# r9y9/wavenet_vocoder

Measured on NVIDIA B200. Metric: audio samples/sec (22.05 kHz MoL, 24-layer), higher is better.
Workload: dtype f32

## Files before the change

### wavenet_vocoder_b200/csrc/wn_host.cu

```cuda
#include <cuda_runtime.h>
#include <stdint.h>
#include <stdio.h>
#include <stdlib.h>
#include <string.h>
#include <math.h>

#include <algorithm>
#include <string>
#include <vector>

#include "../../include/wn.h"
#include "wn_plan.h"
#include "wn_kernel.cuh"
#include "wn7_plan.h"
#include "wn7_kernel.cuh"
#include "wn_aux.cuh"

static thread_local std::string g_err;
static int32_t fail(int32_t code, const std::string& msg) {
    g_err = msg;
    return code;
}
#define CUDA_TRY(expr)                                                                          \
    do {                                                                                        \
// ... 60 lines not shown
    pl.O = c.out_channels;
    pl.kw = c.kernel_size;
    pl.C = c.cin_channels;
    pl.gin = c.gin_channels;
    pl.input_kind = c.input_kind;
    pl.head_kind = c.head_kind;
    pl.Kmix = (c.head_kind == WN_HEAD_SOFTMAX) ? 0 : (c.out_channels == 2 ? 1 : c.out_channels / 3);
    pl.skip_scale = (float)sqrt(1.0 / (double)c.layers);
    pl.BT = batch <= 1 ? 1 : (batch <= 2 ? 2 : (batch <= 4 ? 4 : 8));
    const int BT = pl.BT;

    int P = c.num_ctas > 0 ? c.num_ctas : env_int("WN_NUM_CTAS", 0);
    if (P <= 0) {
        const int cap = std::min(num_sms, pl.G2);
        const int per = wn_ceil_div(pl.G2, cap);
        P = wn_ceil_div(pl.G2, per);
    }
    if (P > num_sms) return fail(WN_ERR_INVALID, "num_ctas exceeds the SM count (blocks must be co-resident)");
    if (P > pl.G2) return fail(WN_ERR_INVALID, "num_ctas exceeds gate_channels/2");
    pl.P = P;
    pl.NYm = wn_ceil_div(pl.G2, P);
    pl.NXm = wn_ceil_div(pl.R, P);
    pl.NSm = wn_ceil_div(pl.S, P);
    pl.NAm = wn_ceil_div(pl.S, P);
    pl.NBm = wn_ceil_div(pl.O, P);
    pl.RA = 2 * pl.NYm;
    pl.NQ_A = wn_ceil_div(pl.RA, 4);
    pl.RA4 = 4 * pl.NQ_A;
    pl.NQ_D = wn_ceil_div((pl.kw - 1) * pl.RA, 4);
    pl.NQ_BO = wn_ceil_div(pl.NXm, 4);
    pl.NQ_BS = wn_ceil_div(pl.NSm, 4);
    pl.NQ_HA = wn_ceil_div(pl.NAm, 4);
    pl.NQ_HB = wn_ceil_div(pl.NBm, 4);
    int o = 0;
    pl.fb_Zx = o; o += pl.NQ_A * pl.R * 4;
    pl.fb_zb = o; o += pl.RA4;
    pl.fb_floats = align_up(o, 4);
    o = 0;
    pl.lb_Zy = o; o += pl.NQ_A * pl.G2 * 4;
    pl.lb_Zx = o; o += pl.NQ_A * pl.R * 4;
    pl.lb_Xo = o; o += pl.NQ_BO * pl.G2 * 4;
    pl.lb_Td = o; o += pl.NQ_D * pl.R * 4;
    pl.lb_Sk = o; o += pl.NQ_BS * pl.G2 * 4;
    pl.lb_zb = o; o += pl.RA4;
    pl.lb_xb = o; o += 4 * pl.NQ_BO;
    pl.lb_sb = o; o += 4 * pl.NQ_BS;
    pl.lb_floats = align_up(o, 4);
    o = 0;
    pl.tb_Td = o;  o += pl.NQ_D * pl.R * 4;
    pl.tb_Sk = o;  o += pl.NQ_BS * pl.G2 * 4;
    pl.tb_sb = o;  o += 4 * pl.NQ_BS;
    pl.tb_Ha = o;  o += pl.NQ_HA * pl.S * 4;
    pl.tb_Hab = o; o += 4 * pl.NQ_HA;
    pl.tb_Hb = o;  o += pl.NQ_HB * pl.S * 4;
    pl.tb_Hbb = o; o += 4 * pl.NQ_HB;
    pl.tb_floats = align_up(o, 4);
    pl.slot_floats = align_up(std::max(pl.fb_floats, std::max(pl.L > 1 ? pl.lb_floats : 0, pl.tb_floats)), 32);
    pl.cta_w_floats = (long long)pl.fb_floats + (long long)(pl.L - 1) * pl.lb_floats + pl.tb_floats;
    pl.nblobs = pl.L + 1;
    pl.cta_cw_floats = (long long)pl.L * pl.NQ_A * pl.C * 4;

    pl.NE = pl.L + 3;
    int nc = c.exchange_copies > 0 ? c.exchange_copies : env_int("WN_NCOPY", 0);
    const int max_items = std::max(std::max(pl.NYm, pl.NXm), std::max(pl.NSm, std::max(pl.NAm, pl.NBm))) * BT;
    if (max_items > 64) return fail(WN_ERR_INVALID, "too many rows per block for this batch tile (use more blocks)");
    if (nc <= 0) nc = 1;
// ... 165 lines not shown
    const int R = pl.R, G2 = pl.G2, kw = pl.kw, S = pl.S, L = pl.L;
    auto grow = [&](int rr) { return (rr & 1) ? G2 + y0 + (rr >> 1) : y0 + (rr >> 1); };
    auto pack_taps = [&](float* grp, int layer) {
        const float* cw = w.layers[layer].conv_w;
        for (int rr = 0; rr < 2 * ny; ++rr)
            for (int tap = 0; tap < kw - 1; ++tap)
                for (int k = 0; k < R; ++k)
                    put_q(grp, R, tap * pl.RA + rr, k, cw[(size_t)grow(rr) * kw * R + (size_t)tap * R + k]);
    };
    auto pack_skip = [&](float* grp, float* bias, int layer) {
        const wn_layer_weights& lw = w.layers[layer];
        for (int r = 0; r < ns; ++r) {
            for (int k = 0; k < G2; ++k) put_q(grp, G2, r, k, lw.skip_w[(size_t)(s0 + r) * G2 + k]);
            bias[r] = lw.skip_b ? lw.skip_b[s0 + r] : 0.f;
        }
    };
    {
        float* blob = out;
        for (int rr = 0; rr < 2 * ny; ++rr) {
            for (int k = 0; k < R; ++k) put_q(blob + pl.fb_Zx, R, rr, k, f.V[0][(size_t)grow(rr) * R + k]);
            blob[pl.fb_zb + rr] = f.zb[0][grow(rr)];
        }
    }
    for (int s = 1; s < L; ++s) {
        float* blob = out + wn_blob_off(pl, s);
        const wn_layer_weights& pw = w.layers[s - 1];
        for (int rr = 0; rr < 2 * ny; ++rr) {
            const int g = grow(rr);
            for (int k = 0; k < G2; ++k) put_q(blob + pl.lb_Zy, G2, rr, k, f.M[s - 1][(size_t)g * G2 + k]);
            for (int k = 0; k < R; ++k) put_q(blob + pl.lb_Zx, R, rr, k, f.V[s][(size_t)g * R + k]);
            blob[pl.lb_zb + rr] = f.zb[s][g];
        }
        for (int r = 0; r < nx; ++r) {
            for (int k = 0; k < G2; ++k) put_q(blob + pl.lb_Xo, G2, r, k, pw.out_w[(size_t)(x0 + r) * G2 + k]);
            blob[pl.lb_xb + r] = pw.out_b ? pw.out_b[x0 + r] : 0.f;
        }
        pack_taps(blob + pl.lb_Td, s - 1);
        pack_skip(blob + pl.lb_Sk, blob + pl.lb_sb, s - 1);
    }
    float* tb = out + wn_blob_off(pl, L);
    pack_taps(tb + pl.tb_Td, L - 1);
    pack_skip(tb + pl.tb_Sk, tb + pl.tb_sb, L - 1);
    for (int r = 0; r < na; ++r) {
        const float* row = w.last_a_w + (size_t)(a0 + r) * S;
        for (int k = 0; k < S; ++k) put_q(tb + pl.tb_Ha, S, r, k, row[k]);
        tb[pl.tb_Hab + r] = w.last_a_b ? w.last_a_b[a0 + r] : 0.f;
    }
    for (int r = 0; r < nb; ++r) {
        const float* row = w.last_b_w + (size_t)(b0 + r) * S;
        for (int k = 0; k < S; ++k) put_q(tb + pl.tb_Hb, S, r, k, row[k]);
        tb[pl.tb_Hbb + r] = w.last_b_b ? w.last_b_b[b0 + r] : 0.f;
    }
}

static void pack_cw_cta(const WnPlan& pl, const wn_weights& w, int p, float* out) {
    if (pl.C <= 0) return;
    memset(out, 0, (size_t)pl.cta_cw_floats * sizeof(float));
    int y0, ny;
    wn_part(pl.G2, pl.P, p, y0, ny);
    for (int l = 0; l < pl.L; ++l) {
        const float* cwm = w.layers[l].cond_w;
        float* grp = out + (size_t)l * pl.NQ_A * pl.C * 4;
        for (int j = 0; j < ny; ++j)
            for (int ab = 0; ab < 2; ++ab) {
                const int rr = 2 * j + ab, grow = ab ? pl.G2 + y0 + j : y0 + j;
                for (int ch = 0; ch < pl.C; ++ch) put_q(grp, pl.C, rr, ch, cwm[(size_t)grow * pl.C + ch]);
            }
    }
// ... 130 lines not shown
    pp.T = T;
    pp.T_test = Tt;
    pp.initial_index = a->initial_index < 0 ? 127 : a->initial_index;
    pp.flags = a->flags;
    pp.noise_kind = a->noise_kind;
    pp.seed = a->seed;
    pp.timeout_cycles = (long long)env_int("WN_TIMEOUT_MS", 2000) * 1500000LL;
    pp.warp_reverse = env_int("WN_WARP_REVERSE", 0);
    pp.gate_cycles = env_int("WN_GATE_CYCLES", 0);
    pp.fast_gate = env_int("WN_FAST_GATE", 0);
    pp.prof = nullptr;
    if (env_int("WN_PROF", 0)) {
        const size_t pb = (size_t)pl.P * 16 * sizeof(long long);
        rc = ensure(&h->d_prof, &h->prof_bytes, pb);
        if (rc) return rc;
        CUDA_TRY(cudaMemsetAsync(h->d_prof, 0, pb, st));
        pp.prof = h->d_prof;
    }

    void* kargs[2] = {(void*)&pl, (void*)&pp};
    auto efor = [](int K) { return K <= 128 ? 1 : (K <= 256 ? 2 : (K <= 512 ? 4 : 8)); };
    const int er = efor(pl.R), eg = efor(pl.G2);
    const int var = (er == 1 && eg == 1) ? 0 : ((er <= 2 && eg <= 2) ? 1 : ((er <= 4 && eg <= 2) ? 2 : 3));
    {
        static const int evar[4][2] = {{1, 1}, {2, 2}, {4, 2}, {8, 8}};
        const int chunk = 1 << pl.xc_shift;
        pl.lean = (BT == 1 && (var == 1 || var == 2) && pl.ncopy == 1 && pl.kw == 3 && pl.RA == 4 && pl.NQ_A == 1 && pl.NQ_BO == 1 && pl.NQ_BS == 1 &&
                   pl.NQ_D == 2 && pl.L >= 2 && evar[var][0] * 128 == pl.R && evar[var][1] * 128 == pl.G2 &&
                   (evar[var][0] % 2) == 0 && (evar[var][1] % 2) == 0 && (pl.ex_yx % chunk) == 0 &&
                   ((pl.G2 + pl.R) % chunk) == 0 && (pl.G2 % chunk) == 0 && (pl.xstride % 2) == 0 &&
                   pl.S == pl.G2 && pl.NQ_HA == 1 && pl.NQ_HB == 1 && pl.O <= 128 && (pl.ex_sk % chunk) == 0 &&
                   (pl.ex_h1 % chunk) == 0 &&
                   env_int("WN_LEAN", 0) != 0) ? 1 : 0;
    }
    const void* fn = nullptr;
#define WN_PICK(BT_)                                                                          \
    fn = var == 0 ? (const void*)wn::wn_persistent_kernel<BT_, 1, 1>                          \
       : var == 1 ? (const void*)wn::wn_persistent_kernel<BT_, 2, 2>                          \
       : var == 2 ? (const void*)wn::wn_persistent_kernel<BT_, 4, 2>                          \
                  : (const void*)wn::wn_persistent_kernel<BT_, 8, 8>
    switch (BT) {
        case 1: WN_PICK(1); break;
        case 2: WN_PICK(2); break;
        case 4: WN_PICK(4); break;
        default: WN_PICK(8); break;
    }
#undef WN_PICK
    if (pl.lean)
        fn = var == 1 ? (const void*)wn::wn_persistent_kernel<1, 2, 2, true>
                      : (const void*)wn::wn_persistent_kernel<1, 4, 2, true>;
    const int ai = pl.lean ? 16 + var : bt_index(BT) * 4 + var;
    if (!h->attr_set[ai]) {
        CUDA_TRY(cudaFuncSetAttribute(fn, cudaFuncAttributeMaxDynamicSharedMemorySize, (int)h->smem_cap));
        h->attr_set[ai] = true;
    }
    cudaLaunchConfig_t lc;
    memset(&lc, 0, sizeof(lc));
    lc.gridDim = dim3(pl.P);
    lc.blockDim = dim3(WN_NTHREADS);
    lc.dynamicSmemBytes = (size_t)pl.smem_bytes;
    lc.stream = st;
    cudaLaunchAttribute la[2];
    int na = 0;
    la[na].id = cudaLaunchAttributeCooperative;
    la[na].val.cooperative = 1;
    ++na;
    if (h->l2_mode == 1 && h->l2_persist_bytes > 0 && h->wpack_bytes > 0) {
        const size_t win = std::min(h->wpack_bytes, h->l2_window_max);
        la[na].id = cudaLaunchAttributeAccessPolicyWindow;
        la[na].val.accessPolicyWindow.base_ptr = (void*)h->d_wpack;
        la[na].val.accessPolicyWindow.num_bytes = win;
        la[na].val.accessPolicyWindow.hitRatio = (float)std::min(1.0, (double)h->l2_persist_bytes / (double)win);
        la[na].val.accessPolicyWindow.hitProp = cudaAccessPropertyPersisting;
        la[na].val.accessPolicyWindow.missProp = cudaAccessPropertyStreaming;
        ++na;
    } else if (h->l2_mode == 2 && h->l2_persist_bytes > 0) {
        la[na].id = cudaLaunchAttributeAccessPolicyWindow;
        la[na].val.accessPolicyWindow.base_ptr = (void*)h->d_xbuf;
        la[na].val.accessPolicyWindow.num_bytes = std::min(xb, h->l2_window_max);
        la[na].val.accessPolicyWindow.hitRatio = 1.0f;
        la[na].val.accessPolicyWindow.hitProp = cudaAccessPropertyPersisting;
        la[na].val.accessPolicyWindow.missProp = cudaAccessPropertyNormal;
        ++na;
    }
// ... 740 lines not shown
```

### wavenet_vocoder_b200/csrc/wn_kernel.cuh

```cuda
#pragma once
#include <cuda_runtime.h>
#include <stdint.h>
#include <math.h>
#include "wn_plan.h"

struct WnPtrs {
    const float* wpack;
    const float* cwpack;
    const float* gbias;
    const float* first_w;
    const float* first_b;
    uint2* xbuf;
    float* ring_g;
    const int* ringtab;
    int* err;
    const float* c;
    const float* initial;
    const float* initial_dense;
    const int* initial_rows;
    const float* test_scalar;
    const int* test_index;
    const float* test_dense;
    const float* u1;
    const float* u2;
// ... 37 lines not shown
    asm volatile(
        "{\n\t.reg .pred p;\n\t"
        "mbarrier.try_wait.parity.shared::cta.b64 p, [%1], %2;\n\t"
        "selp.u32 %0, 1, 0, p;\n\t}"
        : "=r"(ok)
        : "r"(smem_u32(bar)), "r"(parity)
        : "memory");
    return ok != 0;
}
__device__ __forceinline__ void bulk_g2s(void* dst, const void* src, uint32_t bytes, uint64_t* bar) {
    asm volatile(
        "cp.async.bulk.shared::cluster.global.mbarrier::complete_tx::bytes [%0], [%1], %2, [%3];" ::"r"(
            smem_u32(dst)),
        "l"(src), "r"(bytes), "r"(smem_u32(bar))
        : "memory");
}
__device__ __forceinline__ uint2 ld_pair(const uint2* p) {
    uint2 v;
    asm volatile("ld.relaxed.gpu.global.v2.u32 {%0,%1}, [%2];" : "=r"(v.x), "=r"(v.y) : "l"(p) : "memory");
    return v;
}
__device__ __forceinline__ uint4 ld_pair2(const uint2* p) {
    uint4 v;
    asm volatile("ld.relaxed.gpu.global.v4.u32 {%0,%1,%2,%3}, [%4];"
                 : "=r"(v.x), "=r"(v.y), "=r"(v.z), "=r"(v.w)
                 : "l"(p)
                 : "memory");
    return v;
}
__device__ __forceinline__ void st_pair(uint2* p, float v, uint32_t tag) {
    asm volatile("st.relaxed.gpu.global.v2.u32 [%0], {%1,%2};" ::"l"(p), "r"(__float_as_uint(v)), "r"(tag)
                 : "memory");
}
__device__ __forceinline__ void fence_cta() { asm volatile("fence.acq_rel.cta;" ::: "memory"); }
__device__ __forceinline__ int ld_flag(const int* p) {
    int v;
    asm volatile("ld.relaxed.gpu.global.s32 %0, [%1];" : "=r"(v) : "l"(p) : "memory");
    return v;
}
__device__ __forceinline__ bool bar_or(bool pred) {
    uint32_t r;
    asm volatile(
        "{\n\t.reg .pred p, q;\n\t"
        "setp.ne.u32 p, %1, 0;\n\t"
        "bar.red.or.pred q, 1, %2, p;\n\t"
        "selp.u32 %0, 1, 0, q;\n\t}"
        : "=r"(r)
        : "r"((uint32_t)pred), "n"(WN_NT)
        : "memory");
    return r != 0;
}

template <int ID, int N>
__device__ __forceinline__ bool bar_or_n(bool pred) {
    uint32_t r;
    asm volatile(
        "{\n\t.reg .pred p, q;\n\t"
        "setp.ne.u32 p, %1, 0;\n\t"
        "bar.red.or.pred q, %2, %3, p;\n\t"
        "selp.u32 %0, 1, 0, q;\n\t}"
        : "=r"(r)
        : "r"((uint32_t)pred), "n"(ID), "n"(N)
        : "memory");
    return r != 0;
}

// ... 112 lines not shown
    }
    return false;
}
__device__ __noinline__ bool wn_wait_bar_slow(uint64_t* bar, uint32_t parity, volatile int* s_abort, int* err,
                                              long long timeout, uint32_t what, int p) {
    uint32_t spins = 0;
    long long t0 = 0;
    while (!mbar_try_wait(bar, parity)) {
        if (((++spins) & 255u) == 0 && wn_check_abort(s_abort, err, timeout, what, p, t0)) return false;
    }
    return true;
}
__device__ __noinline__ bool wn_wait_count_slow(volatile int* cnt, int need, unsigned sleep_ns, volatile int* s_abort,
                                                int* err, long long timeout, uint32_t what, int p) {
    uint32_t spins = 0;
    long long t0 = 0;
    while (*cnt < need) {
        if (sleep_ns) __nanosleep(sleep_ns);
        if (((++spins) & 63u) == 0 && wn_check_abort(s_abort, err, timeout, what, p, t0)) return false;
    }
    return true;
}

#define WN_NTC 128
#define WN_GW 4
#define WN_DISPATCH_E(EV, ...)                                \
    switch (EV) {                                             \
        case 1: { constexpr int E = 1; __VA_ARGS__ } break;   \
        case 2: { constexpr int E = 2; __VA_ARGS__ } break;   \
        case 4: { constexpr int E = 4; __VA_ARGS__ } break;   \
        default: { constexpr int E = 8; __VA_ARGS__ } break;  \
    }

template <int BT, int ER, int EG, bool LEAN = false>
struct Engine {
    static_assert(!LEAN || (BT == 1 && ER % 2 == 0 && EG % 2 == 0), "lean path: one utterance, paired elements");
    static constexpr int NV = 4 * BT;
    static constexpr int NA = (BT >= 8) ? 1 : 2;
    const WnPlan& pl;
    const WnPtrs& pp;
    unsigned char* sm;
    int tid, warp, lane, p;
    int gt, gw;
    uint64_t *bar_full, *bar_empty, *bar_cfull, *bar_cempty;
    volatile int* s_abort;
    volatile int* s_stash_cnt;
    volatile int* s_ddone_cnt;
    int* ringtab;
    float *xs, *ys, *red1, *red2, *sb, *pre, *cond, *skipacc, *hs, *noise, *first, *slots;
    volatile float* ring;
    float* s_in;
    int* s_idx;
    float* s_dense;
    bool dead;

    __device__ Engine(const WnPlan& pl_, const WnPtrs& pp_, unsigned char* sm_)
        : pl(pl_), pp(pp_), sm(sm_) {
        lane = threadIdx.x & 31;
        warp = pp.warp_reverse ? (WN_NTHREADS / 32 - 1) - (int)(threadIdx.x >> 5) : (int)(threadIdx.x >> 5);
        tid = warp * 32 + lane;
        p = blockIdx.x;
        gt = tid & (WN_NTC - 1);
        gw = warp & (WN_GW - 1);
        const int nslots = pl.nres + pl.nring;
        bar_full = reinterpret_cast<uint64_t*>(sm + pl.sm_bar);
        bar_empty = bar_full + nslots;
        bar_cfull = bar_empty + (pl.nring > 0 ? pl.nring : 1);
        bar_cempty = bar_cfull + 2;
        s_abort = reinterpret_cast<volatile int*>(sm + pl.sm_misc);
// ... 96 lines not shown
#pragma unroll
                    for (int b = 0; b < BT; ++b) x[j][b] = 0.f;
                }
            }
        }
        return bad;
    }
    template <int E>
    __device__ __forceinline__ void poll_vec(const uint2* __restrict__ src, int e0, int K, uint32_t tag,
                                             float (&x)[E][BT]) {
        uint32_t spins = 0;
        long long t0 = 0;
        while (load_vec<E>(src, e0, K, tag, x) != 0) {
            if (((++spins) & 63u) == 0 && check_abort(tag, t0)) {
                dead = true;
                return;
            }
        }
    }
    template <int EA, int EB>
    __device__ __forceinline__ void poll_vec2(const uint2* __restrict__ src, int ea, int KA, float (&a)[EA][BT],
                                              int eb, int KB, float (&b)[EB][BT], uint32_t tag) {
        uint32_t spins = 0;
        long long t0 = 0;
        while (true) {
            const uint32_t bad = load_vec<EA>(src, ea, KA, tag, a) | load_vec<EB>(src, eb, KB, tag, b);
            if (bad == 0) return;
            if (((++spins) & 63u) == 0 && check_abort(tag, t0)) {
                dead = true;
                return;
            }
        }
    }
    template <int E>
    __device__ __forceinline__ void stash(float* dst, int K, const float (&x)[E][BT]) {
#pragma unroll
        for (int j = 0; j < E; ++j) {
            const int k = elem<E>(j);
            if (k < K) {
#pragma unroll
                for (int b = 0; b < BT; ++b) dst[k * BT + b] = x[j][b];
            }
        }
    }
    template <int E>
    __device__ __forceinline__ void unstash(const float* src, int K, float (&x)[E][BT]) {
#pragma unroll
        for (int j = 0; j < E; ++j) {
            const int k = elem<E>(j);
#pragma unroll
            for (int b = 0; b < BT; ++b) x[j][b] = (k < K) ? src[k * BT + b] : 0.f;
        }
    }

    template <int E>
    __device__ __forceinline__ void quad_fma(const float* __restrict__ wq , int K,
                                             const float (&x)[E][BT], float (&acc)[NV]) {
#pragma unroll
        for (int j = 0; j < E; ++j) {
            const int k = elem<E>(j);
            if (k < K) {
                const float4 w4 = *reinterpret_cast<const float4*>(wq + (size_t)k * 4);
#pragma unroll
                for (int b = 0; b < BT; ++b) {
                    acc[0 * BT + b] = fmaf(w4.x, x[j][b], acc[0 * BT + b]);
                    acc[1 * BT + b] = fmaf(w4.y, x[j][b], acc[1 * BT + b]);
// ... 382 lines not shown
            if (lane == 0) mbar_arrive(&bar_cempty[t & 1]);
        }
    }

    __device__ void crit_loop() {
        const int L = pl.L, R = pl.R, G2 = pl.G2, S = pl.S, O = pl.O, T = pp.T, P = pl.P, ncopy = pl.ncopy;
        int y0, ny, x0r, nx, s0, ns, a0, na, b0, nb;
        wn_part(G2, P, p, y0, ny);
        wn_part(R, P, p, x0r, nx);
        wn_part(S, P, p, s0, ns);
        wn_part(S, P, p, a0, na);
        wn_part(O, P, p, b0, nb);
        const int ES = efor(S), EO = efor(O);
        const uint2* xin = pp.xbuf + (size_t)(p % ncopy) * pl.copy_stride_pairs;
        const uint32_t NEID = (uint32_t)L + 3u;
        const int YX = G2 + R;
        const float RSQRT2 = 0.70710678118654752440f;
        const int NQ_A = pl.NQ_A, NQ_BO = pl.NQ_BO, nqc = NQ_A + NQ_BO;
        const int fl = gt & 63;
        const bool grpA = gt < 64;
        auto role = [&](int nitems, int& item, int& copy) {
            item = -1; copy = 0;
            if (nitems > 0 && fl < nitems * ncopy) { item = fl % nitems; copy = fl / nitems; }
        };
        int it_y, cp_y, it_x, cp_x, it_s, cp_s, it_a, cp_a, it_b, cp_b;
        role(ny * BT, it_y, cp_y);
        role(nx * BT, it_x, cp_x);
        role(ns * BT, it_s, cp_s);
        role(na * BT, it_a, cp_a);
        role(nb * BT, it_b, cp_b);
        if (!grpA) it_y = it_s = it_a = it_b = -1;
        if (grpA) it_x = -1;
        const int pa_idx = it_y >= 0 ? (2 * (it_y / BT)) * BT + (it_y % BT) : 0;
        float xr[ER][BT], yr[EG][BT];
        const bool prof = (pp.prof != nullptr) && tid == 0;
        long long pc[8] = {0, 0, 0, 0, 0, 0, 0, 0}, tc = 0;
#define WN_TICK(i) if (prof) { const long long now_ = clock64(); pc[i] += now_ - tc; tc = now_; }
        int nstash = 0;
        int ndone = 0;
        long long t_pub = clock64();
        if (bar_groups(false)) return;

        constexpr bool LEAN_T = LEAN;
        constexpr bool lean = LEAN;
        constexpr int LY = LEAN_T ? EG / 2 : 1, LX = LEAN_T ? ER / 2 : 1;
        long long lk_y[LY], lk_x[LX], l_inc = 0;
        const uint2* l_in0 = xin;
        uint2 *l_puby = pp.xbuf, *l_pubx = pp.xbuf;
        const float* l_pre = pre;
        const uint2 *l_sk0 = xin, *l_h10 = xin;
        uint2 *l_pubs = pp.xbuf, *l_puba = pp.xbuf, *l_pubb = pp.xbuf;
        int l_zy = 0, l_zx = 0, l_xo = 0, l_redw = 0, l_reda = 0, l_redx = 0, l_xb = 0, l_xs = 0;
#pragma unroll
        for (int j = 0; j < LY; ++j) lk_y[j] = 0;
#pragma unroll
        for (int j = 0; j < LX; ++j) lk_x[j] = 0;
        if (lean) {
#pragma unroll
            for (int j = 0; j < LY; ++j) lk_y[j] = wn_pair_index((long long)(2 * gt + 2 * WN_NTC * j));
#pragma unroll
            for (int j = 0; j < LX; ++j) lk_x[j] = wn_pair_index((long long)(G2 + 2 * gt + 2 * WN_NTC * j));
            l_inc = wn_pair_index((long long)YX);
            l_in0 = xin + wn_pair_index((long long)pl.ex_yx);
            l_puby = pp.xbuf + wn_pair_index((long long)pl.ex_yx) + wn_pair_index((long long)(y0 + max(it_y, 0)));
            l_pubx = pp.xbuf + wn_pair_index((long long)pl.ex_yx) + wn_pair_index((long long)(G2 + x0r + max(it_x, 0)));
            l_pre = pre + 2 * max(it_y, 0);
            l_zy = pl.lb_Zy + 8 * gt;
            l_zx = pl.lb_Zx + 8 * gt;
            l_xo = pl.lb_Xo + 8 * gt;
            l_redw = (lane >> 2) * WN_GW + gw;
            l_reda = 2 * max(it_y, 0) * WN_GW;
            l_redx = (4 + max(it_x, 0)) * WN_GW;
            l_xb = pl.lb_xb + max(it_x, 0);
            l_xs = x0r + max(it_x, 0);
            l_sk0 = xin + wn_pair_index((long long)pl.ex_sk);
            l_h10 = xin + wn_pair_index((long long)pl.ex_h1);
            l_pubs = pp.xbuf + wn_pair_index((long long)(pl.ex_sk + s0 + max(it_s, 0)));
            l_puba = pp.xbuf + wn_pair_index((long long)(pl.ex_h1 + a0 + max(it_a, 0)));
            l_pubb = pp.xbuf + wn_pair_index((long long)(pl.ex_h2 + b0 + max(it_b, 0)));
        }
        auto lean_poll_y = [&](const uint2* base, uint32_t tag) {
            uint4 ry[LY];
            uint32_t need = (1u << LY) - 1u, spins = 0;
            while (true) {
#pragma unroll
                for (int j = 0; j < LY; ++j)
                    if (need & (1u << j)) ry[j] = ld_pair2(base + lk_y[j]);
#pragma unroll
                for (int j = 0; j < LY; ++j)
                    if (((ry[j].y ^ tag) | (ry[j].w ^ tag)) == 0u) need &= ~(1u << j);
                if (need == 0u) break;
                if (((++spins) & 63u) == 0 && wn_poll_check(s_abort, pp.err, spins, pp.timeout_cycles, tag, p)) {
                    dead = true;
                    break;
                }
            }
#pragma unroll
            for (int j = 0; j < LY; ++j) {
                yr[2 * j][0] = __uint_as_float(ry[j].x);
                yr[2 * j + 1][0] = __uint_as_float(ry[j].z);
            }
        };
        auto lean_poll_x = [&](const uint2* base, uint32_t tag) {
            uint4 rx[LX];
            uint32_t need = (1u << LX) - 1u, spins = 0;
            while (true) {
#pragma unroll
// ... 112 lines not shown
                                const float yv = yr[j][0];
                                a4[0] = fmaf(wy[j].x, yv, a4[0]); a4[1] = fmaf(wy[j].y, yv, a4[1]);
                                a4[2] = fmaf(wy[j].z, yv, a4[2]); a4[3] = fmaf(wy[j].w, yv, a4[3]);
                            }
                            reduce_scatter<4>(a4, lane);
                            float* r1 = red1 + (s & 1) * pl.red1_floats;
                            if ((lane & 7) == 0) r1[(lane >> 3) * WN_GW + gw] = a4[0];
#pragma unroll
                            for (int j = 0; j < LY; ++j)
                                *reinterpret_cast<float2*>(yst + 2 * gt + 2 * WN_NTC * j) = make_float2(yr[2 * j][0], yr[2 * j + 1][0]);
                            if (bar_or_n<1, WN_NTC>(dead)) { step_dead = true; break; }
                            if (gt == 0) {
                                fence_cta();
                                *s_stash_cnt = nstash + 1;
                            }
                            ++nstash;
                            WN_TICK(1);
                            if (it_y >= 0) {
                                const float a = quad_sum(r1 + l_reda) + pre_a;
                                const float g = quad_sum(r1 + l_reda + WN_GW) + pre_b;
                                st_pair(l_puby + (long long)s * l_inc, pp.fast_gate ? gate_fast(a, g) : gate(a, g), tag + 1u);
                            }
                            release_blob(t, s);
                            if (pp.gate_cycles > 0) t_pub = clock64();
                            if (s >= 2) { count_lean(s_ddone_cnt, WN_GW * (ndone + 1), 0u, 0x08000000u); ++ndone; }
                            WN_TICK(3);
                        }
                    }
                }
                for (int s = s_next; s < L; ++s) {
                    const float* W = acquire_blob(t, s);
                    float pre_a = 0.f, pre_b = 0.f;
                    if (it_y >= 0) { pre_a = pre[pa_idx + s * pl.RA4 * BT]; pre_b = pre[pa_idx + s * pl.RA4 * BT + BT]; }
                    WN_TICK(4);
                    {
                        const int e0 = pl.ex_yx + (s - 1) * YX;
                        const uint32_t tag = tagbase + wn_eid_yx(s - 1);
                        if (pp.gate_cycles > 0) { while (clock64() - t_pub < pp.gate_cycles) {} }
                        if (s >= 2) poll_vec2<EG, ER>(xin, e0, G2, yr, e0 + G2, R, xr, tag);
                        else poll_vec<EG>(xin, e0, G2, tag, yr);
                    }
                    WN_TICK(0);
                    float* xst = xs + (size_t)(s & 1) * R * BT;
                    float* r1 = red1 + (size_t)(s & 1) * pl.red1_floats;
                    stash<ER>(xst, R, xr);
                    stash<EG>(ys + (size_t)(s & 1) * G2 * BT, G2, yr);
                    for (int q = 0; q < nqc; q += NA) {
                        float acc[NA][NV];
#pragma unroll
                        for (int h = 0; h < NA; ++h) {
#pragma unroll
                            for (int v = 0; v < NV; ++v) acc[h][v] = 0.f;
                            const int qq = q + h;
                            if (qq < NQ_A) {
                                quad_fma<EG>(W + pl.lb_Zy + (size_t)qq * G2 * 4, G2, yr, acc[h]);
                                quad_fma<ER>(W + pl.lb_Zx + (size_t)qq * R * 4, R, xr, acc[h]);
                            } else if (qq < nqc) {
                                quad_fma<EG>(W + pl.lb_Xo + (size_t)(qq - NQ_A) * G2 * 4, G2, yr, acc[h]);
                            }
                        }
                        reduce_scatter_multi<NA, NV>(acc, lane);
#pragma unroll
                        for (int h = 0; h < NA; ++h)
                            if (q + h < nqc) quad_store(acc[h], q + h, r1);
                    }
                    WN_TICK(1);
                    if (bar_or_n<1, WN_NTC>(dead)) { step_dead = true; break; }
                    if (gt == 0) {
                        __threadfence_block();
                        *s_stash_cnt = nstash + 1;
                    }
                    ++nstash;
                    WN_TICK(2);
                    const uint32_t tag = tagbase + wn_eid_yx(s);
                    if (it_y >= 0) {
                        const int fr = it_y / BT, fb = it_y % BT;
                        const float a = red_sum(r1, 2 * fr, fb) + pre_a;
                        const float g = red_sum(r1, 2 * fr + 1, fb) + pre_b;
                        publish(pl.ex_yx + s * YX + y0 + fr, fb, cp_y, gate(a, g), tag);
                    }
                    if (it_x >= 0) {
                        const int fr = it_x / BT, fb = it_x % BT;
                        const float o = red_sum(r1, NQ_A * 4 + fr, fb) + W[pl.lb_xb + fr];
                        publish(pl.ex_yx + s * YX + G2 + x0r + fr, fb, cp_x, (o + xst[(x0r + fr) * BT + fb]) * RSQRT2, tag);
                    }
                    release_blob(t, s);
                    t_pub = clock64();
                    if (s >= 2) { wait_count(s_ddone_cnt, WN_GW * (ndone + 1), 0x08000000u); ++ndone; }
                    WN_TICK(3);
                }
                if (step_dead) break;
                bool tail_done = false;
                if constexpr (LEAN_T) {
                    if (lean) {
                        tail_done = true;
                        const float* H = acquire_lean(t, L);
                        lean_poll_x(l_in0 + (long long)(L - 1) * l_inc, tagbase + (uint32_t)(L - 1));
                        lean_poll_y(l_in0 + (long long)(L - 1) * l_inc, tagbase + (uint32_t)(L - 1));
                        WN_TICK(0);
                        float* xst = xs + (L & 1) * R;
#pragma unroll
                        for (int j = 0; j < LX; ++j)
                            *reinterpret_cast<float2*>(xst + 2 * gt + 2 * WN_NTC * j) = make_float2(xr[2 * j][0], xr[2 * j + 1][0]);
                        float* r1 = red1 + (L & 1) * pl.red1_floats;
                        float* r1a = red1 + ((L + 1) & 1) * pl.red1_floats;
                        {
                            float a4[4] = {0.f, 0.f, 0.f, 0.f};
                            lean_quad_y(H + pl.tb_Sk + 8 * gt, a4);
                            reduce_scatter<4>(a4, lane);
                            if ((lane & 7) == 0) r1[(lane >> 3) * WN_GW + gw] = a4[0];
                        }
                        WN_TICK(1);
                        if (bar_or_n<1, WN_NTC>(dead)) { step_dead = true; break; }
                        if (gt == 0) {
                            fence_cta();
                            *s_stash_cnt = nstash + 1;
                        }
// ... 5 lines not shown
                            float tot = quad_sum(r1 + it_s * WN_GW) + H[pl.tb_sb + it_s];
                            tot = skipacc[it_s] + tot;
                            st_pair(l_pubs, fmaxf(tot * pl.skip_scale, 0.f), tagbase + (uint32_t)L);
                        }
                        WN_TICK(3);
                        if (na > 0) {
                            lean_poll_y(l_sk0, tagbase + (uint32_t)L);
                            float a4[4] = {0.f, 0.f, 0.f, 0.f};
                            lean_quad_y(H + pl.tb_Ha + 8 * gt, a4);
                            reduce_scatter<4>(a4, lane);
                            if ((lane & 7) == 0) r1a[(lane >> 3) * WN_GW + gw] = a4[0];
                        }
                        if (bar_or_n<1, WN_NTC>(dead)) { step_dead = true; break; }
                        if (it_a >= 0)
                            st_pair(l_puba, fmaxf(quad_sum(r1a + it_a * WN_GW) + H[pl.tb_Hab + it_a], 0.f), tagbase + (uint32_t)L + 1u);
                        if (nb > 0) {
                            lean_poll_y(l_h10, tagbase + (uint32_t)L + 1u);
                            float a4[4] = {0.f, 0.f, 0.f, 0.f};
                            lean_quad_y(H + pl.tb_Hb + 8 * gt, a4);
                            reduce_scatter<4>(a4, lane);
                            if ((lane & 7) == 0) r1[(lane >> 3) * WN_GW + gw] = a4[0];
                        }
                        if (bar_or_n<1, WN_NTC>(dead)) { step_dead = true; break; }
                        if (it_b >= 0)
                            st_pair(l_pubb, quad_sum(r1 + it_b * WN_GW) + H[pl.tb_Hbb + it_b], tagbase + (uint32_t)L + 2u);
                        release_blob(t, L);
                    }
                }
                if (!tail_done) {
                const float* H = acquire_blob(t, L);
                {
                    const int e0 = pl.ex_yx + (L - 1) * YX;
                    const uint32_t tag = tagbase + wn_eid_yx(L - 1);
                    if (L >= 2) poll_vec2<EG, ER>(xin, e0, G2, yr, e0 + G2, R, xr, tag);
                    else poll_vec<EG>(xin, e0, G2, tag, yr);
                }
                WN_TICK(0);
                stash<ER>(xs + (size_t)(L & 1) * R * BT, R, xr);
                float* r1 = red1 + (size_t)(L & 1) * pl.red1_floats;
                gemv<EG>(H + pl.tb_Sk, pl.NQ_BS, G2, yr, r1);
                WN_TICK(1);
                if (bar_or_n<1, WN_NTC>(dead)) { step_dead = true; break; }
                if (gt == 0) {
                    __threadfence_block();
                    *s_stash_cnt = nstash + 1;
                }
                ++nstash;
                if (L >= 2) { wait_count(s_ddone_cnt, WN_GW * (ndone + 1), 0x08000001u); ++ndone; }
                WN_TICK(2);
                if (it_s >= 0) {
                    const int fr = it_s / BT, fb = it_s % BT;
                    float tot = red_sum(r1, fr, fb) + H[pl.tb_sb + fr];
                    if (L >= 2) tot = skipacc[it_s] + tot;
                    publish(pl.ex_sk + s0 + fr, fb, cp_s, fmaxf(tot * pl.skip_scale, 0.f), tagbase + wn_eid_sk(pl));
                }
                WN_TICK(3);
                float* r1a = red1 + (size_t)((L + 1) & 1) * pl.red1_floats;
                if (na > 0) {
                    WN_DISPATCH_E(ES, { float h[E][BT];
                                        poll_vec<E>(xin, pl.ex_sk, S, tagbase + wn_eid_sk(pl), h);
                                        gemv<E>(H + pl.tb_Ha, pl.NQ_HA, S, h, r1a); });
                }
                if (bar_or_n<1, WN_NTC>(dead)) { step_dead = true; break; }
                if (it_a >= 0) {
                    const int fr = it_a / BT, fb = it_a % BT;
                    publish(pl.ex_h1 + a0 + fr, fb, cp_a, fmaxf(red_sum(r1a, fr, fb) + H[pl.tb_Hab + fr], 0.f), tagbase + wn_eid_h1(pl));
                }
// ... 39 lines not shown
        }
        if (warp < BT) {
            sample_utt(t, warp);
#ifndef WN_NO_SAMPLER_SYNCWARP
            __syncwarp();
#endif
            if (t + 1 < T) fetch_noise(t + 1, warp);
        }
        for (int i = WN_NT - 1 - tid; i < pl.L * (pl.kw - 1); i += WN_NT) {
            const int pos = ringtab[i * 3 + 2] + 1;
            ringtab[i * 3 + 2] = (pos == ringtab[i * 3 + 1]) ? 0 : pos;
        }
    }

    __device__ void def_loop() {
        const int L = pl.L, R = pl.R, G2 = pl.G2, T = pp.T, P = pl.P, kw = pl.kw;
        int s0, ns;
        wn_part(pl.S, P, p, s0, ns);
        const int NQ_D = pl.NQ_D, NQ_BS = pl.NQ_BS, nqd = (kw > 1 ? NQ_D : 0) + NQ_BS;
        const int qoff = (kw > 1 ? NQ_D : 0);
        const int nring_items = (kw - 1) * pl.RA * BT, nskip_items = ns * BT;
        float xr[ER][BT], yr[EG][BT];
        const bool prof = (pp.prof != nullptr) && gt == 0;
        long long pc[4] = {0, 0, 0, 0}, tc = 0;
#define WN_TICK(i) if (prof) { const long long now_ = clock64(); pc[i] += now_ - tc; tc = now_; }
        int nstash = 0;

        constexpr bool LEAN_T = LEAN;
        constexpr bool lean = LEAN;
        const int d_tap = (gt < nring_items) ? gt / pl.RA : 0, d_rr = (gt < nring_items) ? gt % pl.RA : 0;
        int d_x0r, d_nx;
        wn_part(R, P, p, d_x0r, d_nx);
        const int d_fx = (gt >= 64 && gt < 64 + d_nx) ? gt - 64 : -1;
        uint2* d_pubx = pp.xbuf;
        long long d_inc = 0;
        if (lean) {
            d_pubx = pp.xbuf + wn_pair_index((long long)pl.ex_yx) + wn_pair_index((long long)(G2 + d_x0r + max(d_fx, 0)));
            d_inc = wn_pair_index((long long)(G2 + R));
        }
        const float RSQRT2 = 0.70710678118654752440f;
        auto lean_stage = [&](int t, int s, int layer, const float* Td, const float* Sk, const float* skb) -> bool {
            count_lean(s_stash_cnt, nstash + 1, 32u, 0x04000000u);
            ++nstash;
            WN_TICK(0);
            const float* xst = xs + (s & 1) * R;
            const float* yst = ys + (s & 1) * G2;
            float* red = red2 + (s & 1) * pl.red2_floats;
            float accx[4] = {0.f, 0.f, 0.f, 0.f};
            const float* Wb = Sk ? Sk - pl.lb_Sk : nullptr;
            if (Sk) {
                const float* wx = Wb + pl.lb_Xo + 8 * gt;
#pragma unroll
                for (int j = 0; j < EG / 2; ++j) {
                    const float2 yv2 = *reinterpret_cast<const float2*>(yst + 2 * gt + 2 * WN_NTC * j);
#pragma unroll
                    for (int h = 0; h < 2; ++h) {
                        const float4 a = *reinterpret_cast<const float4*>(wx + (2 * WN_NTC * j + h) * 4);
                        const float yv = h ? yv2.y : yv2.x;
                        accx[0] = fmaf(a.x, yv, accx[0]); accx[1] = fmaf(a.y, yv, accx[1]);
                        accx[2] = fmaf(a.z, yv, accx[2]); accx[3] = fmaf(a.w, yv, accx[3]);
                    }
                }
            }
            if (Sk) {
                reduce_scatter<4>(accx, lane);
                if ((lane & 7) == 0) red[(12 + (lane >> 3)) * WN_GW + gw] = accx[0];
                if (bar_or_n<2, WN_NTC>(dead)) dead = true;
                if (!dead && d_fx >= 0) {
                    const float4 q = *reinterpret_cast<const float4*>(red + (12 + d_fx) * WN_GW);
                    const float o = ((q.x + q.y) + (q.z + q.w)) + Wb[pl.lb_xb + d_fx];
                    st_pair(d_pubx + (long long)s * d_inc, (o + xst[d_x0r + d_fx]) * RSQRT2,
                            (uint32_t)t * ((uint32_t)L + 3u) + 1u + (uint32_t)s);
                }
            }
            float acc[8], accs[4];
#pragma unroll
            for (int v = 0; v < 8; ++v) acc[v] = 0.f;
#pragma unroll
            for (int v = 0; v < 4; ++v) accs[v] = 0.f;
            {
                const float *w0 = Td + 8 * gt, *w1 = Td + (size_t)R * 4 + 8 * gt;
#pragma unroll
                for (int j = 0; j < ER / 2; ++j) {
                    const float2 xv2 = *reinterpret_cast<const float2*>(xst + 2 * gt + 2 * WN_NTC * j);
#pragma unroll
                    for (int h = 0; h < 2; ++h) {
                        const int ko = (2 * WN_NTC * j + h) * 4;
                        const float4 a = *reinterpret_cast<const float4*>(w0 + ko);
                        const float4 b = *reinterpret_cast<const float4*>(w1 + ko);
                        const float xv = h ? xv2.y : xv2.x;
                        acc[0] = fmaf(a.x, xv, acc[0]); acc[1] = fmaf(a.y, xv, acc[1]);
                        acc[2] = fmaf(a.z, xv, acc[2]); acc[3] = fmaf(a.w, xv, acc[3]);
                        acc[4] = fmaf(b.x, xv, acc[4]); acc[5] = fmaf(b.y, xv, acc[5]);
                        acc[6] = fmaf(b.z, xv, acc[6]); acc[7] = fmaf(b.w, xv, acc[7]);
                    }
                }
            }
            if (Sk) {
                const float* ws = Sk + 8 * gt;
#pragma unroll
                for (int j = 0; j < EG / 2; ++j) {
                    const float2 yv2 = *reinterpret_cast<const float2*>(yst + 2 * gt + 2 * WN_NTC * j);
#pragma unroll
                    for (int h = 0; h < 2; ++h) {
// ... 82 lines not shown

        build_pre(0);
        if (bar_groups(dead)) return;
        for (int t = 0; t < T; ++t) {
            if (prof) tc = clock64();
            bool step_dead = false;
            release_blob(t, 0);
            for (int s = 1; s < L && !step_dead; ++s) {
                const float* W = acquire_blob(t, s);
                step_dead = stage(t, s, s - 1, W + pl.lb_Td, W + pl.lb_Sk, W + pl.lb_sb);
                release_blob(t, s);
            }
            if (!step_dead) {
                const float* H = acquire_blob(t, L);
                step_dead = stage(t, L, L - 1, H + pl.tb_Td, nullptr, nullptr);
                release_blob(t, L);
            }
            if (!step_dead && t + 1 < T) {
                if (bar_or_n<2, WN_NTC>(dead)) step_dead = true;
                else build_pre(t + 1);
            }
            if (bar_groups(dead || step_dead)) return;
            step_tail(t);
            if (bar_groups(false)) return;
            WN_TICK(3);
        }
        if (prof) {
            for (int i = 0; i < 4; ++i) pp.prof[(size_t)p * 16 + 8 + i] = pc[i];
        }
#undef WN_TICK
    }
};

template <int BT, int ER, int EG, bool LEAN = false>
__global__ void __launch_bounds__(WN_NTHREADS, 1)
wn_persistent_kernel(const __grid_constant__ WnPlan pl, const __grid_constant__ WnPtrs pp) {
    extern __shared__ __align__(1024) unsigned char smem_raw[];
    Engine<BT, ER, EG, LEAN> eng(pl, pp, smem_raw);
    const int tid = eng.tid, p = blockIdx.x;
    const int nslots = pl.nres + pl.nring;
    if (tid == 0) {
        for (int i = 0; i < nslots; ++i) mbar_init(&eng.bar_full[i], 1);
        for (int i = 0; i < pl.nring; ++i) mbar_init(&eng.bar_empty[i], WN_NWARP);
        for (int i = 0; i < 2; ++i) {
            mbar_init(&eng.bar_cfull[i], 1);
            mbar_init(&eng.bar_cempty[i], WN_GW);
        }
        *eng.s_abort = 0;
        *eng.s_stash_cnt = 0;
        *eng.s_ddone_cnt = 0;
        asm volatile("fence.mbarrier_init.release.cluster;" ::: "memory");
    }
    if (pl.ring_in_smem) {
        const size_t n = (size_t)pl.ring_pos_total * pl.RA4 * BT;
        for (size_t i = tid; i < n; i += WN_NTHREADS) eng.ring[i] = 0.f;
    }
    for (int i = tid; i < pl.NSm * BT + 4; i += WN_NTHREADS) eng.skipacc[i] = 0.f;
    for (int i = tid; i < pl.L * (pl.kw - 1); i += WN_NTHREADS) {
        eng.ringtab[i * 3] = pp.ringtab[i * 2];
        eng.ringtab[i * 3 + 1] = pp.ringtab[i * 2 + 1];
        eng.ringtab[i * 3 + 2] = 0;
    }
    for (int k = tid; k < pl.R; k += WN_NTHREADS) {
        eng.first[k] = (pl.input_kind == 0) ? pp.first_w[k] : 0.f;
        eng.first[pl.R + k] = pp.first_b[k];
    }
    {
        int y0, ny;
        wn_part(pl.G2, pl.P, p, y0, ny);
        const float* blob0 = pp.wpack + (size_t)p * pl.cta_w_floats;
        const int n = pl.L * pl.RA4 * BT;
// ... 103 lines not shown
```

### wavenet_vocoder_b200/csrc/wn_plan.h

```cpp
#pragma once
#include <stdint.h>

#ifndef WN_HD
#ifdef __CUDACC__
#define WN_HD __host__ __device__ __forceinline__
#else
#define WN_HD inline
#endif
#endif

#define WN_NT 256
#define WN_NWARP (WN_NT / 32)
#define WN_AUX_WARPS 2
#define WN_NTHREADS (WN_NT + 32 * WN_AUX_WARPS)
#define WN_MAXE 8
#define WN_MAX_BT 8
#define WN_MAX_CI 4

struct WnPlan {
    int L, per_stack, R, G, G2, S, O, kw, C, gin, input_kind, head_kind, Kmix;
    int P;
    int NYm;
    int NXm;
    int NSm;
// ... 1 lines not shown
    int NBm;
    int RA;
    int NQ_A, NQ_D, NQ_BO, NQ_BS, NQ_HA, NQ_HB;
    int fb_Zx, fb_zb, fb_floats;
    int lb_Zy;
    int lb_Zx;
    int lb_Xo;
    int lb_Td;
    int lb_Sk;
    int lb_zb, lb_xb, lb_sb;
    int lb_floats;
    int tb_Td, tb_Sk, tb_sb, tb_Ha, tb_Hab, tb_Hb, tb_Hbb, tb_floats;
    int slot_floats;
    long long cta_w_floats;
    int nblobs;
    int nres;
    int nring;
    long long cta_cw_floats;
    int NE;
    int ncopy;
    int ex_yx, ex_sk, ex_h1, ex_h2, ex_elems;
    long long copy_stride_pairs;
    int BT;
    int ring_in_smem;
    long long ring_pos_total;
    int RA4;
    int sm_bar, sm_misc, sm_ringtab, sm_xs, sm_red1, sm_red2, sm_sb, sm_cond, sm_skipacc, sm_hs,
        sm_noise, sm_in, sm_first, sm_ring, sm_slots, smem_bytes;
    int red1_floats;
    int red2_floats;
    float skip_scale;
    int xc_shift, xstride;
    int lean;
};
WN_HD long long wn_pair_index_(const WnPlan& pl, long long lin) {
    return (long long)(((unsigned long long)lin >> pl.xc_shift) * (unsigned long long)pl.xstride +
                       ((unsigned long long)lin & ((1ull << pl.xc_shift) - 1ull)));
}

WN_HD void wn_part(int rows, int P, int p, int& base, int& cnt) {
    int q = rows / P, r = rows % P;
    base = p * q + (p < r ? p : r);
    cnt = q + (p < r ? 1 : 0);
}

WN_HD int wn_ceil_div(int a, int b) { return (a + b - 1) / b; }
#define WN_XCHUNK 32
#define WN_XSTRIDE 544
#define wn_pair_index(lin) wn_pair_index_(pl, (lin))
WN_HD long long wn_pair_index_(const struct WnPlan& pl, long long lin);
WN_HD int wn_dilation(const WnPlan& pl, int l) { return 1 << (l % pl.per_stack); }
WN_HD int wn_eid_yx(int s) { return s; }
WN_HD int wn_eid_sk(const WnPlan& pl) { return pl.L; }
WN_HD int wn_eid_h1(const WnPlan& pl) { return pl.L + 1; }
WN_HD int wn_eid_h2(const WnPlan& pl) { return pl.L + 2; }
WN_HD long long wn_blob_off(const WnPlan& pl, int i) {
    return i == 0 ? 0 : (long long)pl.fb_floats + (long long)(i - 1) * pl.lb_floats;
}
WN_HD int wn_blob_floats(const WnPlan& pl, int i) {
    return i == 0 ? pl.fb_floats : (i < pl.L ? pl.lb_floats : pl.tb_floats);
}
```

Baseline: 22180.

## Pack per-CTA gate and residual outputs into 128-bit tagged exchange words

Adds an XP kernel variant for P=128, R=512, G/2=256 that permutes residual-row ownership so each CTA's two gate outputs and four residual outputs sit in two adjacent 16-byte words. Each word is published with a single 128-bit relaxed store that carries a tag, and consumers poll two 128-bit words per thread instead of the paired 64-bit loads. The intent is fewer global stores and polls per layer on the latency-bound inter-CTA exchange. In exchange it depends on 128-bit ld/st being atomic with respect to the tag, and it changes the residual row mapping used in host packing and in the lean path.

```diff
diff --git a/wavenet_vocoder_b200/csrc/wn_host.cu b/wavenet_vocoder_b200/csrc/wn_host.cu
--- a/wavenet_vocoder_b200/csrc/wn_host.cu
+++ b/wavenet_vocoder_b200/csrc/wn_host.cu
@@ -116,6 +116,7 @@
     pl.NQ_BS = wn_ceil_div(pl.NSm, 4);
     pl.NQ_HA = wn_ceil_div(pl.NAm, 4);
     pl.NQ_HB = wn_ceil_div(pl.NBm, 4);
+    pl.xrows = (P == 128 && pl.G2 == 2 * P && pl.R == 4 * P) ? 1 : 0;
     int o = 0;
     pl.fb_Zx = o; o += pl.NQ_A * pl.R * 4;
     pl.fb_zb = o; o += pl.RA4;
@@ -347,8 +348,9 @@
             blob[pl.lb_zb + rr] = f.zb[s][g];
         }
         for (int r = 0; r < nx; ++r) {
-            for (int k = 0; k < G2; ++k) put_q(blob + pl.lb_Xo, G2, r, k, pw.out_w[(size_t)(x0 + r) * G2 + k]);
-            blob[pl.lb_xb + r] = pw.out_b ? pw.out_b[x0 + r] : 0.f;
+            const int xr = wn_xrow(pl, p, r);
+            for (int k = 0; k < G2; ++k) put_q(blob + pl.lb_Xo, G2, r, k, pw.out_w[(size_t)xr * G2 + k]);
+            blob[pl.lb_xb + r] = pw.out_b ? pw.out_b[xr] : 0.f;
         }
         pack_taps(blob + pl.lb_Td, s - 1);
         pack_skip(blob + pl.lb_Sk, blob + pl.lb_sb, s - 1);
@@ -545,6 +547,9 @@
                    pl.S == pl.G2 && pl.NQ_HA == 1 && pl.NQ_HB == 1 && pl.O <= 128 && (pl.ex_sk % chunk) == 0 &&
                    (pl.ex_h1 % chunk) == 0 &&
                    env_int("WN_LEAN", 0) != 0) ? 1 : 0;
+        pl.xpack = (pl.xrows && BT == 1 && var == 2 && !pl.lean && pl.ncopy == 1 && pl.L >= 2 && pl.xc_shift >= 1 &&
+                    (pl.xstride % 2) == 0 && (pl.ex_yx % chunk) == 0 && ((pl.G2 + pl.R) % chunk) == 0 &&
+                    env_int("WN_XPACK", 1) != 0) ? 1 : 0;
     }
     const void* fn = nullptr;
 #define WN_PICK(BT_)                                                                          \
@@ -562,7 +567,9 @@
     if (pl.lean)
         fn = var == 1 ? (const void*)wn::wn_persistent_kernel<1, 2, 2, true>
                       : (const void*)wn::wn_persistent_kernel<1, 4, 2, true>;
-    const int ai = pl.lean ? 16 + var : bt_index(BT) * 4 + var;
+    if (pl.xpack)
+        fn = (const void*)wn::wn_persistent_kernel<1, 4, 2, false, true>;
+    const int ai = pl.lean ? 16 + var : pl.xpack ? 19 : bt_index(BT) * 4 + var;
     if (!h->attr_set[ai]) {
         CUDA_TRY(cudaFuncSetAttribute(fn, cudaFuncAttributeMaxDynamicSharedMemorySize, (int)h->smem_cap));
         h->attr_set[ai] = true;
diff --git a/wavenet_vocoder_b200/csrc/wn_kernel.cuh b/wavenet_vocoder_b200/csrc/wn_kernel.cuh
--- a/wavenet_vocoder_b200/csrc/wn_kernel.cuh
+++ b/wavenet_vocoder_b200/csrc/wn_kernel.cuh
@@ -93,6 +93,19 @@
     asm volatile("st.relaxed.gpu.global.v2.u32 [%0], {%1,%2};" ::"l"(p), "r"(__float_as_uint(v)), "r"(tag)
                  : "memory");
 }
+__device__ __forceinline__ uint4 ld_word(const uint2* p) {
+    uint4 v;
+    asm volatile("{\n\t.reg .b128 t;\n\tld.relaxed.gpu.global.b128 t, [%4];\n\tmov.b128 {%0, %1, %2, %3}, t;\n\t}"
+                 : "=r"(v.x), "=r"(v.y), "=r"(v.z), "=r"(v.w)
+                 : "l"(p)
+                 : "memory");
+    return v;
+}
+__device__ __forceinline__ void st_word(uint2* p, float a, float b, float c, uint32_t tag) {
+    asm volatile("{\n\t.reg .b128 t;\n\tmov.b128 t, {%1, %2, %3, %4};\n\tst.relaxed.gpu.global.b128 [%0], t;\n\t}" ::"l"(p),
+                 "r"(__float_as_uint(a)), "r"(__float_as_uint(b)), "r"(__float_as_uint(c)), "r"(tag)
+                 : "memory");
+}
 __device__ __forceinline__ void fence_cta() { asm volatile("fence.acq_rel.cta;" ::: "memory"); }
 __device__ __forceinline__ int ld_flag(const int* p) {
     int v;
@@ -271,9 +284,10 @@
         default: { constexpr int E = 8; __VA_ARGS__ } break;  \
     }
 
-template <int BT, int ER, int EG, bool LEAN = false>
+template <int BT, int ER, int EG, bool LEAN = false, bool XP = false>
 struct Engine {
     static_assert(!LEAN || (BT == 1 && ER % 2 == 0 && EG % 2 == 0), "lean path: one utterance, paired elements");
+    static_assert(!XP || (!LEAN && BT == 1 && ER == 4 && EG == 2), "packed exchange: one utterance, R = 512, G/2 = 256");
     static constexpr int NV = 4 * BT;
     static constexpr int NA = (BT >= 8) ? 1 : 2;
     const WnPlan& pl;
@@ -436,6 +450,29 @@
             }
         }
     }
+    __device__ __forceinline__ void poll_words(const uint2* __restrict__ src, int e0, float (&y)[EG][BT],
+                                               float (&x)[ER][BT], uint32_t tag) {
+        const uint2* wa = src + wn_pair_index((long long)(e0 + 4 * gt));
+        const uint2* wb = src + wn_pair_index((long long)(e0 + 4 * gt + 2));
+        uint32_t spins = 0;
+        long long t0 = 0;
+        uint4 a, b;
+        while (true) {
+            a = ld_word(wa);
+            b = ld_word(wb);
+            if (((a.w ^ tag) | (b.w ^ tag)) == 0u) break;
+            if (((++spins) & 63u) == 0 && check_abort(tag, t0)) {
+                dead = true;
+                break;
+            }
+        }
+        y[0][0] = __uint_as_float(a.x);
+        y[1][0] = __uint_as_float(a.y);
+        x[0][0] = __uint_as_float(a.z);
+        x[1][0] = __uint_as_float(b.x);
+        x[2][0] = __uint_as_float(b.y);
+        x[3][0] = __uint_as_float(b.z);
+    }
     template <int E>
     __device__ __forceinline__ void stash(float* dst, int K, const float (&x)[E][BT]) {
 #pragma unroll
@@ -884,6 +921,13 @@
         if (!grpA) it_y = it_s = it_a = it_b = -1;
         if (grpA) it_x = -1;
         const int pa_idx = it_y >= 0 ? (2 * (it_y / BT)) * BT + (it_y % BT) : 0;
+        const int xg = wn_xrow(pl, p, it_x >= 0 ? it_x / BT : 0);
+        const int xw_fin = XP ? (gt == 0 ? 0 : (gt == 64 ? 1 : -1)) : -1;
+        int xg4[4] = {0, 0, 0, 0};
+        if (XP) {
+#pragma unroll
+            for (int r = 0; r < 4; ++r) xg4[r] = wn_xrow(pl, p, r);
+        }
         float xr[ER][BT], yr[EG][BT];
         const bool prof = (pp.prof != nullptr) && tid == 0;
         long long pc[8] = {0, 0, 0, 0, 0, 0, 0, 0}, tc = 0;
@@ -915,7 +959,7 @@
             l_inc = wn_pair_index((long long)YX);
             l_in0 = xin + wn_pair_index((long long)pl.ex_yx);
             l_puby = pp.xbuf + wn_pair_index((long long)pl.ex_yx) + wn_pair_index((long long)(y0 + max(it_y, 0)));
-            l_pubx = pp.xbuf + wn_pair_index((long long)pl.ex_yx) + wn_pair_index((long long)(G2 + x0r + max(it_x, 0)));
+            l_pubx = pp.xbuf + wn_pair_index((long long)pl.ex_yx) + wn_pair_index((long long)(G2 + xg));
             l_pre = pre + 2 * max(it_y, 0);
             l_zy = pl.lb_Zy + 8 * gt;
             l_zx = pl.lb_Zx + 8 * gt;
@@ -924,7 +968,7 @@
             l_reda = 2 * max(it_y, 0) * WN_GW;
             l_redx = (4 + max(it_x, 0)) * WN_GW;
             l_xb = pl.lb_xb + max(it_x, 0);
-            l_xs = x0r + max(it_x, 0);
+            l_xs = xg;
             l_sk0 = xin + wn_pair_index((long long)pl.ex_sk);
             l_h10 = xin + wn_pair_index((long long)pl.ex_h1);
             l_pubs = pp.xbuf + wn_pair_index((long long)(pl.ex_sk + s0 + max(it_s, 0)));
@@ -1103,12 +1147,15 @@
                     const float* W = acquire_blob(t, s);
                     float pre_a = 0.f, pre_b = 0.f;
                     if (it_y >= 0) { pre_a = pre[pa_idx + s * pl.RA4 * BT]; pre_b = pre[pa_idx + s * pl.RA4 * BT + BT]; }
+                    float4 pre4 = make_float4(0.f, 0.f, 0.f, 0.f);
+                    if (XP && xw_fin == 0) pre4 = *reinterpret_cast<const float4*>(pre + s * pl.RA4);
                     WN_TICK(4);
                     {
                         const int e0 = pl.ex_yx + (s - 1) * YX;
                         const uint32_t tag = tagbase + wn_eid_yx(s - 1);
                         if (pp.gate_cycles > 0) { while (clock64() - t_pub < pp.gate_cycles) {} }
-                        if (s >= 2) poll_vec2<EG, ER>(xin, e0, G2, yr, e0 + G2, R, xr, tag);
+                        if (XP && s >= 2) poll_words(xin, e0, yr, xr, tag);
+                        else if (s >= 2) poll_vec2<EG, ER>(xin, e0, G2, yr, e0 + G2, R, xr, tag);
                         else poll_vec<EG>(xin, e0, G2, tag, yr);
                     }
                     WN_TICK(0);
@@ -1144,16 +1191,31 @@
                     ++nstash;
                     WN_TICK(2);
                     const uint32_t tag = tagbase + wn_eid_yx(s);
-                    if (it_y >= 0) {
-                        const int fr = it_y / BT, fb = it_y % BT;
-                        const float a = red_sum(r1, 2 * fr, fb) + pre_a;
-                        const float g = red_sum(r1, 2 * fr + 1, fb) + pre_b;
-                        publish(pl.ex_yx + s * YX + y0 + fr, fb, cp_y, gate(a, g), tag);
-                    }
-                    if (it_x >= 0) {
-                        const int fr = it_x / BT, fb = it_x % BT;
-                        const float o = red_sum(r1, NQ_A * 4 + fr, fb) + W[pl.lb_xb + fr];
-                        publish(pl.ex_yx + s * YX + G2 + x0r + fr, fb, cp_x, (o + xst[(x0r + fr) * BT + fb]) * RSQRT2, tag);
+                    if constexpr (XP) {
+                        uint2* dst = pp.xbuf + wn_pair_index((long long)(pl.ex_yx + s * YX + 4 * p + 2 * max(xw_fin, 0)));
+                        if (xw_fin == 0) {
+                            const float a0 = red_sum(r1, 0, 0) + pre4.x, g0 = red_sum(r1, 1, 0) + pre4.y;
+                            const float a1 = red_sum(r1, 2, 0) + pre4.z, g1 = red_sum(r1, 3, 0) + pre4.w;
+                            const float o0 = red_sum(r1, NQ_A * 4 + 0, 0) + W[pl.lb_xb + 0];
+                            st_word(dst, gate(a0, g0), gate(a1, g1), (o0 + xst[xg4[0]]) * RSQRT2, tag);
+                        } else if (xw_fin == 1) {
+                            const float o1 = red_sum(r1, NQ_A * 4 + 1, 0) + W[pl.lb_xb + 1];
+                            const float o2 = red_sum(r1, NQ_A * 4 + 2, 0) + W[pl.lb_xb + 2];
+                            const float o3 = red_sum(r1, NQ_A * 4 + 3, 0) + W[pl.lb_xb + 3];
+                            st_word(dst, (o1 + xst[xg4[1]]) * RSQRT2, (o2 + xst[xg4[2]]) * RSQRT2, (o3 + xst[xg4[3]]) * RSQRT2, tag);
+                        }
+                    } else {
+                        if (it_y >= 0) {
+                            const int fr = it_y / BT, fb = it_y % BT;
+                            const float a = red_sum(r1, 2 * fr, fb) + pre_a;
+                            const float g = red_sum(r1, 2 * fr + 1, fb) + pre_b;
+                            publish(pl.ex_yx + s * YX + y0 + fr, fb, cp_y, gate(a, g), tag);
+                        }
+                        if (it_x >= 0) {
+                            const int fr = it_x / BT, fb = it_x % BT;
+                            const float o = red_sum(r1, NQ_A * 4 + fr, fb) + W[pl.lb_xb + fr];
+                            publish(pl.ex_yx + s * YX + G2 + xg, fb, cp_x, (o + xst[xg * BT + fb]) * RSQRT2, tag);
+                        }
                     }
                     release_blob(t, s);
                     t_pub = clock64();
@@ -1225,7 +1287,8 @@
                 {
                     const int e0 = pl.ex_yx + (L - 1) * YX;
                     const uint32_t tag = tagbase + wn_eid_yx(L - 1);
-                    if (L >= 2) poll_vec2<EG, ER>(xin, e0, G2, yr, e0 + G2, R, xr, tag);
+                    if (XP) poll_words(xin, e0, yr, xr, tag);
+                    else if (L >= 2) poll_vec2<EG, ER>(xin, e0, G2, yr, e0 + G2, R, xr, tag);
                     else poll_vec<EG>(xin, e0, G2, tag, yr);
                 }
                 WN_TICK(0);
@@ -1331,10 +1394,11 @@
         int d_x0r, d_nx;
         wn_part(R, P, p, d_x0r, d_nx);
         const int d_fx = (gt >= 64 && gt < 64 + d_nx) ? gt - 64 : -1;
+        const int d_xg = wn_xrow(pl, p, max(d_fx, 0));
         uint2* d_pubx = pp.xbuf;
         long long d_inc = 0;
         if (lean) {
-            d_pubx = pp.xbuf + wn_pair_index((long long)pl.ex_yx) + wn_pair_index((long long)(G2 + d_x0r + max(d_fx, 0)));
+            d_pubx = pp.xbuf + wn_pair_index((long long)pl.ex_yx) + wn_pair_index((long long)(G2 + d_xg));
             d_inc = wn_pair_index((long long)(G2 + R));
         }
         const float RSQRT2 = 0.70710678118654752440f;
@@ -1368,7 +1432,7 @@
                 if (!dead && d_fx >= 0) {
                     const float4 q = *reinterpret_cast<const float4*>(red + (12 + d_fx) * WN_GW);
                     const float o = ((q.x + q.y) + (q.z + q.w)) + Wb[pl.lb_xb + d_fx];
-                    st_pair(d_pubx + (long long)s * d_inc, (o + xst[d_x0r + d_fx]) * RSQRT2,
+                    st_pair(d_pubx + (long long)s * d_inc, (o + xst[d_xg]) * RSQRT2,
                             (uint32_t)t * ((uint32_t)L + 3u) + 1u + (uint32_t)s);
                 }
             }
@@ -1517,11 +1581,11 @@
     }
 };
 
-template <int BT, int ER, int EG, bool LEAN = false>
+template <int BT, int ER, int EG, bool LEAN = false, bool XP = false>
 __global__ void __launch_bounds__(WN_NTHREADS, 1)
 wn_persistent_kernel(const __grid_constant__ WnPlan pl, const __grid_constant__ WnPtrs pp) {
     extern __shared__ __align__(1024) unsigned char smem_raw[];
-    Engine<BT, ER, EG, LEAN> eng(pl, pp, smem_raw);
+    Engine<BT, ER, EG, LEAN, XP> eng(pl, pp, smem_raw);
     const int tid = eng.tid, p = blockIdx.x;
     const int nslots = pl.nres + pl.nring;
     if (tid == 0) {
diff --git a/wavenet_vocoder_b200/csrc/wn_plan.h b/wavenet_vocoder_b200/csrc/wn_plan.h
--- a/wavenet_vocoder_b200/csrc/wn_plan.h
+++ b/wavenet_vocoder_b200/csrc/wn_plan.h
@@ -57,6 +57,8 @@
     float skip_scale;
     int xc_shift, xstride;
     int lean;
+    int xrows;
+    int xpack;
 };
 WN_HD long long wn_pair_index_(const WnPlan& pl, long long lin) {
     return (long long)(((unsigned long long)lin >> pl.xc_shift) * (unsigned long long)pl.xstride +
@@ -70,6 +72,13 @@
 }
 
 WN_HD int wn_ceil_div(int a, int b) { return (a + b - 1) / b; }
+
+WN_HD int wn_xrow(const WnPlan& pl, int p, int r) {
+    if (pl.xrows) return 2 * p + (r & 1) + 2 * pl.P * (r >> 1);
+    int base, cnt;
+    wn_part(pl.R, pl.P, p, base, cnt);
+    return base + r;
+}
 #define WN_XCHUNK 32
 #define WN_XSTRIDE 544
 #define wn_pair_index(lin) wn_pair_index_(pl, (lin))
```

Measured after the change: 17100 (median of 6 runs). 0.771x the previous value.
